# pzimbrod/fem-glass-tempering

Measured on AMD Instinct MI355X. Metric: DOF-updates/sec (coupled thermo-visco time step, 3D CG1 hex), higher is better.
Workload: dtype f64; 1 GPU; C4 3D plate CG1/CG1 400x400x50 hex (8200851 T-dofs), dt 0.1, coupled 6-term Prony; parallelism=single GPU, one partition (no communication), output=none (reference writes VTX/XDMF every step), krylov_form=PETSc KSPCG, geometric-multigrid V-cycle preconditioner, preconditioner=gmg, visco_fields=state (T, Tf, Tf_partial, phi, xi, s_tilde, sigma_tilde, sigma)

## Files before the change

fem-glass-tempering_amd/csrc/tv_cg.hip:

```cpp
#include <algorithm>
#include <cstdlib>

#include "tv_stencil.h"


#include <cstdio>
#include <vector>

namespace tv {
namespace {


using buf_t = __amdgpu_buffer_rsrc_t;
using b64v = unsigned int __attribute__((ext_vector_type(2)));
constexpr uint32_t kBadOff = 0x40000000u;
__device__ __forceinline__ buf_t mk_rsrc(const void* p, uint32_t bytes) {
  const uint64_t a = (uint64_t)p;
  const uint32_t lo = __builtin_amdgcn_readfirstlane((uint32_t)a);
  const uint32_t hi = __builtin_amdgcn_readfirstlane((uint32_t)(a >> 32));
  void* q = (void*)(((uint64_t)hi << 32) | lo);
  return __builtin_amdgcn_make_buffer_rsrc(q, (short)0, (int)__builtin_amdgcn_readfirstlane(bytes), 0x00020000);
}
__device__ __forceinline__ double bload(buf_t r, uint32_t off) {
  return __builtin_bit_cast(double, __builtin_amdgcn_raw_buffer_load_b64(r, (int)off, 0, 0));
}
__device__ __forceinline__ void bstore(buf_t r, uint32_t off, double v) {
  __builtin_amdgcn_raw_buffer_store_b64(__builtin_bit_cast(b64v, v), r, (int)off, 0, 0);
}

__device__ __forceinline__ double uniform(double v) {
  const int lo = __builtin_amdgcn_readfirstlane(__double2loint(v));
  const int hi = __builtin_amdgcn_readfirstlane(__double2hiint(v));
  return __hiloint2double(hi, lo);
}

__device__ __forceinline__ double wave_sum(double v) {
#pragma unroll
  for (int off = 32; off >= 1; off >>= 1) v += __shfl_xor(v, off, 64);
  return v;
}


template <int DIM, int MODE, bool FUSEP>
__global__ __launch_bounds__(kBlock) void k_cg_rows(CgGrid g, const double* __restrict__ T,
                                                    const double* __restrict__ in0,
                                                    const double* in1,
                                                    double* __restrict__ out, double* pout,
                                                    const PcgState* __restrict__ st,
                                                    double* __restrict__ partials, int nseg, int kfirst,
                                                    int nplanes, int wmode) {
  constexpr bool D1 = (DIM <= 2);
  constexpr bool D2 = (DIM == 1);
  __shared__ double red[kBlock / kWave];
  if (st != nullptr && st->done) return;
  const int lane = threadIdx.x & (kWave - 1);
  const int wave = threadIdx.x >> 6;
  int seg, j, kp;
  if (wmode == 0) {
    const int n1b = (g.n1 + 3) >> 2;
    const int b = blockIdx.x;
    seg = b % nseg;
    const int t = b / nseg;
    j = (t % n1b) * 4 + wave;
    kp = t / n1b;
  } else {
    const int gw = blockIdx.x * 4 + wave;
    seg = gw % nseg;
    const int row = gw / nseg;
    j = row % g.n1;
    kp = row / g.n1;
  }
  const int k = kfirst + kp;
  const bool row_ok = (j < g.n1) && (kp < nplanes);
  const int i = seg * kSeg - 1 + lane;
  const bool col_ok = row_ok && (i >= 0) && (i < g.n0);
  const int n0 = g.n0, n1 = g.n1, n2 = g.n2;
  const int64_t plane = (int64_t)n0 * n1;

  double bcoef = 0.0;
  bool first = false;
  const double* pold = in1;
  if (FUSEP) {
    const int it = st->it;
    first = (it == 0);
    bcoef = first ? 0.0 : st->beta / st->betaold;
    if (it & 1) {
      pold = in1;
    } else {
      pold = pout;
      pout = const_cast<double*>(in1);
    }
  }

  double X[3][3];
  double Mm[3][3];
#pragma unroll
  for (int b = 0; b < 3; ++b) {
#pragma unroll
    for (int c = 0; c < 3; ++c) {
      const int jj = j + b - 1, kk = k + c - 1;
      const bool ok = col_ok && (D1 ? b == 1 : (jj >= 0 && jj < n1)) && (D2 ? c == 1 : (kk >= 0 && kk < n2));
      const int64_t idx = (int64_t)i + (int64_t)n0 * jj + plane * kk;
      double v = 0.0, v2 = 0.0;
      if (ok) {
        v = in0[idx];
        if (MODE == MODE_RES) v2 = in1[idx];
        if (FUSEP) v = first ? v : v + bcoef * pold[idx];
      }
      X[b][c] = v;
      if (MODE == MODE_RES) Mm[b][c] = v - v2 - g.dt_f;
    }
  }
  const double* cy = g.coef[1] + (int64_t)(j < n1 ? j : 0) * C_NCOEF;
  const double* cz = g.coef[2] + (int64_t)(k < n2 ? k : 0) * C_NCOEF;
  const double My[3] = {cy[C_MLO], cy[C_MDI], cy[C_MUP]};
  const double Ky[3] = {cy[C_KLO], cy[C_KDI], cy[C_KUP]};
  const double Mz[3] = {cz[C_MLO], cz[C_MDI], cz[C_MUP]};
  const double Kz[3] = {cz[C_KLO], cz[C_KDI], cz[C_KUP]};
  const double da = g.dt_alpha;

  double S1 = 0.0, S2 = 0.0;
#pragma unroll
  for (int c = 0; c < 3; ++c) {
    double us = 0.0, vs = 0.0, um = 0.0;
#pragma unroll
    for (int b = 0; b < 3; ++b) {
      us += My[b] * X[b][c];
      vs += Ky[b] * X[b][c];
      if (MODE == MODE_RES) um += My[b] * Mm[b][c];
    }
    if (MODE != MODE_RES) um = us;
    S1 += Mz[c] * (um + da * vs) + da * Kz[c] * us;
    S2 += Mz[c] * us;
  }
  S2 *= da;

  const double S1m = shr1(S1), S1p = shl1(S1), S2m = shr1(S2), S2p = shl1(S2);
  const double* cx = g.coef[0] + (int64_t)(col_ok ? i : 0) * C_NCOEF;
  double y = 0.0;
  if (col_ok) {
    y = cx[C_MLO] * S1m + cx[C_MDI] * S1 + cx[C_MUP] * S1p + cx[C_KLO] * S2m + cx[C_KDI] * S2 +
        cx[C_KUP] * S2p;
  }

  if (!D2 && row_ok && ((k == 0 && g.bnd[2][0]) || (k == n2 - 1 && g.bnd[2][1]))) {
    double Tp_[3][3], Pp_[3][3];
#pragma unroll
    for (int v = 0; v < 3; ++v) {
      double pc = X[v][1], tc;
      if (MODE == MODE_RES) {
        tc = pc;
      } else {
        const int jj = j + v - 1;
        const bool ok = col_ok && (D1 ? v == 1 : (jj >= 0 && jj < n1));
        tc = ok ? T[(int64_t)i + (int64_t)n0 * jj + plane * k] : 0.0;
      }
      Tp_[0][v] = shr1(tc); Tp_[1][v] = tc; Tp_[2][v] = shl1(tc);
      Pp_[0][v] = shr1(pc); Pp_[1][v] = pc; Pp_[2][v] = shl1(pc);
    }
    if (col_ok) {
      y += facet_sum<MODE, false, false, D1>(g, cx[C_HLO], cx[C_HHI], cy[C_HLO], cy[C_HHI], Tp_, Pp_);
    }
  }
  if (!D1 && row_ok && ((j == 0 && g.bnd[1][0]) || (j == n1 - 1 && g.bnd[1][1]))) {
    double Tp_[3][3], Pp_[3][3];
#pragma unroll
    for (int v = 0; v < 3; ++v) {
      double pc = X[1][v], tc;
      if (MODE == MODE_RES) {
        tc = pc;
      } else {
        const int kk = k + v - 1;
        const bool ok = col_ok && (D2 ? v == 1 : (kk >= 0 && kk < n2));
        tc = ok ? T[(int64_t)i + (int64_t)n0 * j + plane * kk] : 0.0;
      }
      Tp_[0][v] = shr1(tc); Tp_[1][v] = tc; Tp_[2][v] = shl1(tc);
      Pp_[0][v] = shr1(pc); Pp_[1][v] = pc; Pp_[2][v] = shl1(pc);
    }
    if (col_ok) {
      y += facet_sum<MODE, false, false, D2>(g, cx[C_HLO], cx[C_HHI], cz[C_HLO], cz[C_HHI], Tp_, Pp_);
    }
  }
  if (col_ok && ((i == 0 && g.bnd[0][0]) || (i == n0 - 1 && g.bnd[0][1]))) {
    double Tp_[3][3];
    if (MODE == MODE_RES) {
#pragma unroll
      for (int u = 0; u < 3; ++u)
#pragma unroll
        for (int v = 0; v < 3; ++v) Tp_[u][v] = X[u][v];
    } else {
#pragma unroll
      for (int u = 0; u < 3; ++u) {
#pragma unroll
        for (int v = 0; v < 3; ++v) {
          const int jj = j + u - 1, kk = k + v - 1;
          const bool ok = (D1 ? u == 1 : (jj >= 0 && jj < n1)) && (D2 ? v == 1 : (kk >= 0 && kk < n2));
          Tp_[u][v] = ok ? T[(int64_t)i + (int64_t)n0 * jj + plane * kk] : 0.0;
        }
      }
    }
    y += facet_sum<MODE, false, D1, D2>(g, cy[C_HLO], cy[C_HHI], cz[C_HLO], cz[C_HHI], Tp_, X);
  }

  const bool owned = (k >= g.k_begin) && (k < g.k_end);
  const bool inwin = (k >= g.w_begin) && (k < g.w_end);
  const bool writer = col_ok && lane >= 1 && lane <= kSeg;
  const int64_t me = (int64_t)i + (int64_t)n0 * j + plane * k;
  if (writer) {
    if (FUSEP) pout[me] = X[1][1];
    if (inwin) out[me] = y;
  }
  if (MODE == MODE_JAC && partials != nullptr) {
    double d = (writer && owned) ? X[1][1] * y : 0.0;
    d = wave_sum(d);
    if (lane == 0) red[wave] = d;
    __syncthreads();
    if (threadIdx.x == 0) store_partial(&partials[blockIdx.x], (red[0] + red[1]) + (red[2] + red[3]));
  }
}


template <int DIM, bool FACETS>
__device__ __forceinline__ double diag_value(const CgGrid& g, const double* __restrict__ T, int64_t n) {
  constexpr bool D1 = (DIM <= 2);
  constexpr bool D2 = (DIM == 1);
  const int64_t plane = (int64_t)g.n0 * g.n1;
  int i, j, k;
  decode_node(n, g, i, j, k);
  const double* cx = g.coef[0] + (int64_t)i * C_NCOEF;
  const double* cy = g.coef[1] + (int64_t)j * C_NCOEF;
  const double* cz = g.coef[2] + (int64_t)k * C_NCOEF;
  double d = cx[C_MDI] * cy[C_MDI] * cz[C_MDI] +
             g.dt_alpha * (cx[C_KDI] * cy[C_MDI] * cz[C_MDI] + cx[C_MDI] * cy[C_KDI] * cz[C_MDI] +
                           cx[C_MDI] * cy[C_MDI] * cz[C_KDI]);
  if (!FACETS) return d;
  auto load_patch = [&](int64_t stride_a, int64_t stride_b, bool dega, bool degb, int ia, int na, int ib, int nb,
                        double (&P)[3][3]) {
#pragma unroll
    for (int u = 0; u < 3; ++u)
#pragma unroll
      for (int v = 0; v < 3; ++v) {
        const int aa = ia + u - 1, bb = ib + v - 1;
        const bool ok = (dega ? u == 1 : (aa >= 0 && aa < na)) && (degb ? v == 1 : (bb >= 0 && bb < nb));
        P[u][v] = ok ? T[n + (int64_t)(u - 1) * stride_a + (int64_t)(v - 1) * stride_b] : 0.0;
      }
  };
  double P[3][3];
  if ((i == 0 && g.bnd[0][0]) || (i == g.n0 - 1 && g.bnd[0][1])) {
    load_patch(g.n0, plane, D1, D2, j, g.n1, k, g.n2, P);
    d += facet_sum<MODE_JAC, true, D1, D2>(g, cy[C_HLO], cy[C_HHI], cz[C_HLO], cz[C_HHI], P, P);
  }
  if (!D1 && ((j == 0 && g.bnd[1][0]) || (j == g.n1 - 1 && g.bnd[1][1]))) {
    load_patch(1, plane, false, D2, i, g.n0, k, g.n2, P);
    d += facet_sum<MODE_JAC, true, false, D2>(g, cx[C_HLO], cx[C_HHI], cz[C_HLO], cz[C_HHI], P, P);
  }
  if (!D2 && ((k == 0 && g.bnd[2][0]) || (k == g.n2 - 1 && g.bnd[2][1]))) {
    load_patch(1, g.n0, false, D1, i, g.n0, j, g.n1, P);
    d += facet_sum<MODE_JAC, true, false, D1>(g, cx[C_HLO], cx[C_HHI], cy[C_HLO], cy[C_HHI], P, P);
  }
  return d;
}

template <int DIM, bool FACETS>
__global__ __launch_bounds__(kBlock) void k_cg_diag(CgGrid g, const double* __restrict__ T,
                                                    double* __restrict__ out, int invert) {
  const int64_t plane = (int64_t)g.n0 * g.n1;
  const int64_t nown = plane * (g.w_end - g.w_begin);
  const int64_t base = plane * g.w_begin;
  for (int64_t t = blockIdx.x * (int64_t)blockDim.x + threadIdx.x; t < nown;
       t += (int64_t)gridDim.x * blockDim.x) {
    const int64_t n = base + t;
    const double d = diag_value<DIM, FACETS>(g, T, n);
    out[n] = invert ? 1.0 / d : d;
  }
}

__global__ __launch_bounds__(kBlock) void k_cg_diag_bnd(CgGrid g, const double* __restrict__ T,
                                                        double* __restrict__ out, int invert) {
  for (int64_t t = blockIdx.x * (int64_t)blockDim.x + threadIdx.x; t < g.n_bnodes;
       t += (int64_t)gridDim.x * blockDim.x) {
    const int64_t n = g.bnodes[t];
    const double d = diag_value<3, true>(g, T, n);
    out[n] = invert ? 1.0 / d : d;
  }
}


constexpr int kRows = 8;
constexpr int kFaceChunk = 16;

template <int MODE, bool FUSEP>
__device__ double facet_direct(const CgGrid& g, int i, int j, int k, int ax, const double* __restrict__ T,
                               const double* __restrict__ in0, const double* pold, double bcoef, bool first) {
  const int t1 = (ax == 0) ? 1 : 0, t2 = (ax == 2) ? 1 : 2;
  const int c[3] = {i, j, k};
  const int n[3] = {g.n0, g.n1, g.n2};
  const int64_t st[3] = {1, g.n0, (int64_t)g.n0 * g.n1};
  const int64_t me = (int64_t)i + st[1] * j + st[2] * k;
  double Tp[3][3], Pp[3][3];
#pragma unroll
  for (int u = 0; u < 3; ++u)
#pragma unroll
    for (int v = 0; v < 3; ++v) {
      const int a = c[t1] + u - 1, b = c[t2] + v - 1;
      const bool ok = a >= 0 && a < n[t1] && b >= 0 && b < n[t2];
      const int64_t off = me + (int64_t)(u - 1) * st[t1] + (int64_t)(v - 1) * st[t2];
      if (MODE == MODE_RES) {
        Tp[u][v] = ok ? in0[off] : 0.0;
        Pp[u][v] = 0.0;
      } else {
        Tp[u][v] = ok ? T[off] : 0.0;
        double pv = ok ? in0[off] : 0.0;
        if (FUSEP && ok && !first) pv = pv + bcoef * pold[off];
        Pp[u][v] = pv;
      }
    }
  const double* c1 = g.coef[t1] + (int64_t)c[t1] * C_NCOEF;
  const double* c2 = g.coef[t2] + (int64_t)c[t2] * C_NCOEF;
  return facet_sum<MODE, false, false, false>(g, c1[C_HLO], c1[C_HHI], c2[C_HLO], c2[C_HHI], Tp, Pp);
}

struct FaceOff {
  int off[7];
};

FaceOff face_offsets(const CgGrid& g, int R, int qaxis) {
  FaceOff fo{};
  int acc = 0;
  const int rows = R - 1;
  for (int f = 0; f < 6; ++f) {
    fo.off[f] = acc;
    if (g.fface[f] && (f >> 1) != qaxis) acc += ((g.fn1[f] + kSeg - 1) / kSeg) * ((g.fn2[f] + rows - 1) / rows);
  }
  fo.off[6] = acc;
  return fo;
}

__device__ __forceinline__ void facet_corners(const CgGrid& g, bool ok, double h1, double h2, double Ta,
                                              double Tc, double Pa, double Pc, double& ya, double& yb,
                                              double& yc, double& yd) {
  const double Tb = shl1(Ta), Td = shl1(Tc), Pb = shl1(Pa), Pd = shl1(Pc);
  ya = yb = yc = yd = 0.0;
  if (ok) {
#pragma unroll
    for (int q1 = 0; q1 < 3; ++q1) {
#pragma unroll
      for (int q2 = 0; q2 < 3; ++q2) {
        const double sx = kGX[q1], tx = kGX[q2];
        const double fa = (1.0 - sx) * (1.0 - tx), fb = sx * (1.0 - tx), fc = (1.0 - sx) * tx, fd = sx * tx;
        const double Th = fa * Ta + fb * Tb + fc * Tc + fd * Td;
        const double Ph = fa * Pa + fb * Pb + fc * Pc + fd * Pd;
        const double G = (kGW[q1] * kGW[q2]) * dg_rad_conv(g, Th) * Ph;
        ya += G * fa;
        yb += G * fb;
        yc += G * fc;
        yd += G * fd;
      }
    }
    const double sc = g.dt * (h1 * h2);
    ya *= sc; yb *= sc; yc *= sc; yd *= sc;
  }
}

template <bool FUSEP, int R>
__device__ void face_block(const CgGrid& g, const double* __restrict__ T, const double* __restrict__ in0,
                           const double* pA, const double* pB, double beta_ratio,
                           double* __restrict__ partials, const RedTail& rt, int nrec, int fb,
                           const FaceOff& fo, double* sm, double* redf, int it_host) {
  double (*sT)[kWave] = reinterpret_cast<double (*)[kWave]>(sm);
  double (*sP)[kWave] = reinterpret_cast<double (*)[kWave]>(sm + (R + 1) * kWave);
  double (*sCD)[R][kWave] = reinterpret_cast<double (*)[R][kWave]>(sm + 2 * (R + 1) * kWave);
  int f = 0;
  while (f < 5 && fb >= fo.off[f + 1]) ++f;
  const int a = f >> 1, side = f & 1;
  const int t1 = (a == 0) ? 1 : 0, t2 = (a == 2) ? 1 : 2;
  const int n[3] = {g.n0, g.n1, g.n2};
  const int sst[3] = {1, g.n0, g.n0 * g.n1};
  const int n1 = n[t1], n2 = n[t2];
  const int nseg1 = (n1 + kSeg - 1) / kSeg;
  const int tile = fb - fo.off[f];
  const int seg = tile % nseg1, tb = tile / nseg1;
  const int lane = threadIdx.x & (kWave - 1);
  const int wave = __builtin_amdgcn_readfirstlane(threadIdx.x >> 6);
  const int c1 = seg * kSeg - 1 + lane;
  const int r0 = tb * (R - 1);
  const bool ok1 = c1 >= 0 && c1 < n1;
  double bcoef = 0.0;
  bool first = true;
  const double* pold = pA;
  if (FUSEP) {
    first = (it_host == 0);
    bcoef = first ? 0.0 : beta_ratio;
    pold = (it_host & 1) ? pA : pB;
  }
  auto node_of = [&](int cc1, int cc2) {
    int c[3];
    c[t1] = cc1;
    c[t2] = cc2;
    c[a] = side ? n[a] - 1 : 0;
    return c[0] + sst[1] * c[1] + sst[2] * c[2];
  };
  struct Stg {
    double tt, zz, oo;
    bool ok;
  };
  auto stage_ld = [&](int cc2) -> Stg {
    const bool ok = ok1 && cc2 >= 0 && cc2 < n2;
    const int o = ok ? node_of(c1, cc2) : 0;
    return Stg{T[o], in0[o], FUSEP ? pold[o] : 0.0, ok};
  };
  auto stage_st = [&](int row, const Stg& v) {
    sT[row][lane] = v.ok ? v.tt : 0.0;
    sP[row][lane] = v.ok ? ((FUSEP && !first) ? v.zz + bcoef * v.oo : v.zz) : 0.0;
  };
  const int fr = r0 - 1 + wave;
  const bool facet_ok = c1 >= 0 && c1 < n1 - 1 && fr >= 0 && fr < n2 - 1;
  const double h1 = g.coef[t1][(int64_t)(facet_ok ? c1 : 0) * C_NCOEF + C_HHI];
  const double h2 = g.coef[t2][(int64_t)(facet_ok ? fr : 0) * C_NCOEF + C_HHI];
  const Stg sa = stage_ld(r0 - 1 + wave);
  Stg sb{0.0, 0.0, 0.0, false};
  if (wave == R - 1) sb = stage_ld(r0 + R - 1);
  stage_st(wave, sa);
  if (wave == R - 1) stage_st(R, sb);
  __syncthreads();
  const double Pa = sP[wave][lane];
  double ya, yb, yc, yd;
  facet_corners(g, facet_ok, h1, h2, sT[wave][lane], sT[wave + 1][lane], Pa, sP[wave + 1][lane], ya, yb, yc, yd);
  sCD[0][wave][lane] = yc;
  sCD[1][wave][lane] = yd;
  const double ybl = shr1(yb);
  __syncthreads();
  double dot = 0.0;
  const int c2 = r0 - 1 + wave;
  const bool wr = wave >= 1 && ok1 && lane >= 1 && lane <= kSeg && c2 < n2;
  if (wr) {
    const double acc = (ya + ybl) + (sCD[0][wave - 1][lane] + sCD[1][wave - 1][lane - 1]);
    int c[3];
    c[t1] = c1;
    c[t2] = c2;
    c[a] = side ? n[a] - 1 : 0;
    const bool owned = c[2] >= g.k_begin && c[2] < g.k_end;
    g.fface[f][c1 + n1 * c2] = (c[2] >= g.w_begin && c[2] < g.w_end) ? acc : 0.0;
    dot = owned ? Pa * acc : 0.0;
  }
  if (partials != nullptr) {
    dot = wave_sum(dot);
    if (lane == 0) redf[wave] = dot;
    __syncthreads();
    if (threadIdx.x == 0) {
      double s2 = 0.0;
#pragma unroll
      for (int w = 0; w < R; ++w) s2 += redf[w];
      store_partial(&partials[blockIdx.x], s2);
    }
    fused_reduce_tail<1>(rt, nrec);
  }
}

__global__ __launch_bounds__(kBlock) void k_cg_addfaces(CgGrid g, double* __restrict__ out, int raxis,
                                                        const PcgState* __restrict__ st) {
  if (st != nullptr && st->done) return;
  const int n[3] = {g.n0, g.n1, g.n2};
  const int kb = g.w_begin, nk = g.w_end - g.w_begin;
  const int sx = n[0] > 1 ? 2 : 1;
  const int64_t nA = (int64_t)sx * n[1] * nk;
  const int nin = n[0] - 2 > 0 ? n[0] - 2 : 0;
  const int nfree = (raxis == 1) ? nk : n[1];
  const int64_t nB = 2 * (int64_t)nin * nfree;
  const double* fb = nullptr;
#pragma unroll
  for (int f = 0; f < 6; ++f)
    if (fb == nullptr && g.fface[f] != nullptr) fb = g.fface[f] - g.ffoff[f];
  const buf_t rsF = mk_rsrc(fb, fb ? (uint32_t)(g.ffsize * 8) : 0u);
  const uint32_t obytes = (uint32_t)n[0] * (uint32_t)n[1] * (uint32_t)n[2] * 8u;
  const buf_t rsO = mk_rsrc(out, obytes);
  const int fr_lo = (raxis == 1) ? 2 : 4;
  for (int64_t e = blockIdx.x * (int64_t)kBlock + threadIdx.x; e < nA + nB; e += (int64_t)gridDim.x * kBlock) {
    int c[3];
    if (e < nA) {
      const int64_t pl = (int64_t)n[1] * nk;
      const int side = (int)(e / pl);
      const int64_t r = e - side * pl;
      c[0] = side ? n[0] - 1 : 0;
      c[1] = (int)(r % n[1]);
      c[2] = kb + (int)(r / n[1]);
    } else {
      const int64_t u = e - nA, pl = (int64_t)nin * nfree;
      const int side = (int)(u / pl);
      const int64_t r = u - side * pl;
      c[0] = 1 + (int)(r % nin);
      const int o = (int)(r / nin);
      if (raxis == 1) {
        c[1] = side ? n[1] - 1 : 0;
        c[2] = kb + o;
      } else {
        c[1] = o;
        c[2] = side ? n[2] - 1 : 0;
        if (c[2] < kb || c[2] >= g.w_end) continue;
      }
    }
    const bool x0 = g.fface[0] && c[0] == 0, x1 = g.fface[1] && c[0] == n[0] - 1;
    const bool r0 = g.fface[fr_lo] && c[raxis] == 0, r1 = g.fface[fr_lo + 1] && c[raxis] == n[raxis] - 1;
    const int rt2 = (raxis == 1) ? c[2] : c[1];
    const int64_t ex = (x0 ? g.ffoff[0] : g.ffoff[1]) + c[1] + (int64_t)n[1] * c[2];
    const int64_t er = (r0 ? g.ffoff[fr_lo] : g.ffoff[fr_lo + 1]) + c[0] + (int64_t)n[0] * rt2;
    const uint32_t oq = (uint32_t)(c[0] + (int64_t)n[0] * (c[1] + (int64_t)n[1] * c[2])) * 8u;
    const double fx = bload(rsF, (x0 || x1) ? (uint32_t)ex * 8u : kBadOff);
    const double fr = bload(rsF, (r0 || r1) ? (uint32_t)er * 8u : kBadOff);
    const double old = bload(rsO, oq);
    const double add = fx + fr;
    if (add != 0.0) bstore(rsO, oq, old + add);
  }
}

__device__ __forceinline__ void march_tile(int bid, int nmarch, int nseg, int nrbk, int nch, int& seg, int& rb,
                                           int& chunk) {
  const int x = bid & 7, p = bid >> 3;
  const int q = nmarch >> 3, r = nmarch & 7;
  const int start = x * q + min(x, r);
  const int per_chunk = nseg * nrbk;
  const int nF = (nch > 1 ? 2 : 1) * per_chunk;
  const int fq = nF >> 3, fr = nF & 7;
  const int fsize = fq + (x < fr ? 1 : 0), fstart = x * fq + min(x, fr);
  int t, c;
  if (p < fsize) {
    t = fstart + p;
    c = t / per_chunk;
    chunk = c ? nch - 1 : 0;
  } else {
    t = (start - fstart) + (p - fsize);
    c = t / per_chunk;
    chunk = 1 + c;
  }
  t -= c * per_chunk;
  seg = t % nseg;
  rb = t / nseg;
}

template <int MODE, bool FUSEP, int R, int WPE, int PF, bool POST = false>
__global__ __launch_bounds__(R * kWave) __attribute__((amdgpu_waves_per_eu(WPE))) void k_cg_march(CgGrid g, const double* __restrict__ T,
                                                        const double* __restrict__ in0, const double* in1,
                                                        double* __restrict__ out, double* pout,
                                                        const PcgState* __restrict__ st,
                                                        double* __restrict__ partials, int nseg, int raxis,
                                                        int qchunk, RedTail rt, int nrec, int nmarch,
                                                        FaceOff fo, int it_host, PostArgs pa) {
  static_assert(!POST || (MODE == MODE_JAC && !FUSEP), "POST: plain Jacobian march only");
  stamp_start(rt);
  constexpr int NA = (MODE == MODE_RES) ? 2 : 1;
  __shared__ double lds[NA][2][R + 2][kWave];
  __shared__ double red[R];
  constexpr int kFaceLds = (MODE == MODE_JAC) ? (8 * R + 8) * kWave : 1;
  __shared__ double fsm[kFaceLds];
  const int bid = (int)blockIdx.x;
  const int fidx = (MODE == MODE_JAC && bid >= nmarch) ? bid - nmarch : -1;
  const bool lagged = FUSEP && rt.lag != nullptr;
  if (lagged && bid == 0 && threadIdx.x == 0) {
    const PcgState s = lagged_state(st, rt.lag, rt.lag_kind);
    if (s.done) *rt.st = s;
  }
  if (fidx >= 0) {
    double ratio = 0.0;
    if (lagged) {
      int ldone;
      double lbeta;
      lag_update_lean(st, rt.lag, ldone, lbeta);
      if (ldone) return;
      ratio = lbeta / st->betaold;
    } else if (st != nullptr) {
      if (st->done) return;
      if (FUSEP) ratio = st->beta / st->betaold;
    }
    face_block<FUSEP, R>(g, T, in0, in1, pout, ratio, POST ? nullptr : partials, POST ? RedTail{} : rt, nrec, fidx, fo,
                         fsm, red, it_host);
    return;
  }
  const int lane = threadIdx.x & (kWave - 1);
  const int wave = __builtin_amdgcn_readfirstlane(threadIdx.x >> 6);
  const int n0 = g.n0;
  const int nR = (raxis == 1) ? g.n1 : g.n2;
  const int nQ = (raxis == 1) ? g.n2 : g.n1;
  const int64_t sR = (raxis == 1) ? (int64_t)n0 : (int64_t)n0 * g.n1;
  const int64_t sQ = (raxis == 1) ? (int64_t)n0 * g.n1 : (int64_t)n0;
  const int nch = (nQ + qchunk - 1) / qchunk;
  const int nrbk = (nR + R - 1) / R;
  int seg, rb, chunk;
  march_tile(bid, nmarch, nseg, nrbk, nch, seg, rb, chunk);
  const int r0 = rb * R;
  const int r = r0 + wave;
  const bool row_ok = r < nR;
  const int q0 = chunk * qchunk;
  const int q1 = min(q0 + qchunk, nQ);
  const int i = seg * kSeg - 1 + lane;
  const bool col_ok = (i >= 0) && (i < n0);
  const bool writer = col_ok && lane >= 1 && lane <= kSeg;

  double bcoef = 0.0;
  bool first = false;
  const double* pold = in1;
  if (FUSEP) {
    first = (it_host == 0);
    if (!(it_host & 1)) { pold = pout; pout = const_cast<double*>(in1); }
  }
  int st_done = 0;
  double st_beta = 0.0, st_betaold = 1.0;
  if (lagged) {
    lag_update_lean(st, rt.lag, st_done, st_beta);
    st_done = __builtin_amdgcn_readfirstlane(st_done);
    st_beta = uniform(st_beta);
    st_betaold = st->betaold;
  } else if (st != nullptr) {
    st_done = st->done;
    if (FUSEP) {
      st_beta = st->beta;
      st_betaold = st->betaold;
    }
  }
  const int kb = g.k_begin, ke = g.k_end, wb = g.w_begin, we = g.w_end;
  const bool row_owned = (raxis == 2) ? (r >= kb && r < ke) : true;
  const bool row_inwin = (raxis == 2) ? (r >= wb && r < we) : true;
  const double* coefR = (raxis == 1) ? g.coef[1] : g.coef[2];
  const double* coefQ = (raxis == 1) ? g.coef[2] : g.coef[1];
  const int bq_lo = (raxis == 1) ? g.bnd[2][0] : g.bnd[1][0];
  const int bq_hi = (raxis == 1) ? g.bnd[2][1] : g.bnd[1][1];

  const bool fq0 = (MODE == MODE_JAC) && q0 == 0 && bq_lo;
  const bool fq1 = (MODE == MODE_JAC) && q1 == nQ && bq_hi;
  double (*sFq)[2][R + 2][kWave] = reinterpret_cast<double (*)[2][R + 2][kWave]>(fsm);
  double (*sCD)[2][R][kWave] = reinterpret_cast<double (*)[2][R][kWave]>(fsm + 4 * (R + 2) * kWave);
  double yq0 = 0.0, yq1 = 0.0;
  const double da = g.dt_alpha;

  const double* second = (MODE == MODE_RES) ? in1 : pold;
  constexpr bool TWO = (MODE == MODE_RES) || FUSEP;
  const uint32_t nbytes = (uint32_t)g.n0 * (uint32_t)g.n1 * (uint32_t)g.n2 * 8u;
  const buf_t rs0 = mk_rsrc(in0, nbytes);
  const buf_t rs1 = mk_rsrc(TWO ? second : in0, (FUSEP && first) ? 0u : nbytes);
  const buf_t rso = mk_rsrc(out, nbytes);
  const buf_t rsp = mk_rsrc(FUSEP ? pout : out, FUSEP ? nbytes : 0u);
  const buf_t rsT = mk_rsrc(T, (fq0 || fq1) ? nbytes : 0u);
  const buf_t rsZ = mk_rsrc(in0, (fq0 || fq1) ? nbytes : 0u);
  const buf_t rsO = mk_rsrc(TWO ? second : in0, ((fq0 || fq1) && FUSEP && !first) ? nbytes : 0u);
  const bool halo = (wave == 0) || (wave == R - 1);
  const int hrow = (wave == 0) ? r0 - 1 : (wave == R - 1 ? r0 + R : r);
  const int hslot = (wave == 0) ? 0 : R + 1;
  auto lane_off = [&](int rr) -> uint32_t {
    return (col_ok && rr >= 0 && rr < nR) ? (uint32_t)(i + sR * rr) * 8u : kBadOff;
  };
  const uint32_t vo_own = lane_off(r), vo_halo = halo ? lane_off(hrow) : kBadOff;
  const uint32_t vo_wr = writer ? vo_own : kBadOff;
  auto plane_off = [&](int L) -> uint32_t { return (L >= 0 && L < nQ) ? (uint32_t)(sQ * L) * 8u : kBadOff; };
  auto fetch = [&](uint32_t vo, int L, double& a0, double& a1) {
    const uint32_t o = vo + plane_off(L);
    a0 = bload(rs0, o);
    a1 = TWO ? bload(rs1, o) : 0.0;
  };
  const buf_t rsr = mk_rsrc(pa.r, POST ? nbytes : 0u);
  const buf_t rsd = mk_rsrc(pa.dinv, POST ? nbytes : 0u);
  const int bR_lo = (raxis == 1) ? g.bnd[1][0] : g.bnd[2][0], bR_hi = (raxis == 1) ? g.bnd[1][1] : g.bnd[2][1];
  const bool bnd_lr = (i == 0) || (i == n0 - 1) || (r == 0 && bR_lo) || (r == nR - 1 && bR_hi);
  auto bnd_q = [&](int q) { return (q == 0 && bq_lo) || (q == nQ - 1 && bq_hi); };
  auto fetch_post = [&](int L, double& a_r, double& a_d) {
    if (!POST) return;
    const uint32_t o = vo_wr + plane_off(L - 1);
    a_r = bload(rsr, o);
    a_d = bload(rsd, (bnd_lr || bnd_q(L - 1)) ? o : kBadOff);
  };

  auto combine = [&](uint32_t vo, int L, double a0, double a1, double& v, double& vm) {
    v = a0;
    vm = 0.0;
    if (MODE == MODE_RES) vm = (vo != kBadOff && L >= 0 && L < nQ) ? a0 - a1 - g.dt_f : 0.0;
    if (FUSEP) v = a0 + bcoef * a1;
  };
  double ra0[PF + 1], ra1[PF + 1], rh0[PF + 1], rh1[PF + 1];
  double rr[PF + 1], rd[PF + 1];
#pragma unroll
  for (int s = 0; s < PF; ++s) {
    fetch(vo_own, q0 - 1 + s, ra0[s], ra1[s]);
    fetch(vo_halo, q0 - 1 + s, rh0[s], rh1[s]);
    fetch_post(q0 - 1 + s, rr[s], rd[s]);
  }
  __shared__ double2 cql[kFaceChunk + 2][5];
  __shared__ double2 cxl[4][kWave];
  __shared__ double crl[R + 1][C_NCOEF];
  const int nqs = q1 - q0 + 2;
  const bool st_q = (int)threadIdx.x < nqs * 6;
  const bool st_x = (int)threadIdx.x < 8 * kWave;
  const bool st_r = (int)threadIdx.x < (R + 1) * C_NCOEF;
  double cqv, cxv, crv;
  {
    const int e = threadIdx.x;
    const int qq = q0 - 1 + e / 6;
    const bool okq = st_q && qq >= 0 && qq < nQ;
    cqv = coefQ[okq ? (int64_t)qq * C_NCOEF + e % 6 : 0];
    const int ii = seg * kSeg - 1 + (e & (kWave - 1));
    const bool okx = st_x && ii >= 0 && ii < n0;
    const int k = e >> 6;
    const int cc = k == 0 ? C_MLO : k == 1 ? C_KLO : k == 2 ? C_MDI : k == 3 ? C_KDI : k == 4 ? C_MUP : k == 5 ? C_KUP : C_HHI;
    cxv = g.coef[0][okx ? (int64_t)ii * C_NCOEF + cc : 0];
    const int rrow = r0 - 1 + e / C_NCOEF;
    const bool okr = st_r && rrow >= 0 && rrow < nR;
    crv = coefR[okr ? (int64_t)rrow * C_NCOEF + e % C_NCOEF : 0];
    cqv = okq ? cqv : 0.0;
    cxv = (okx && k < 7) ? cxv : 0.0;
    crv = okr ? crv : 0.0;
  }
  double fT[2][2], fZ[2][2], fO[2][2];
  if (fq0 || fq1) {
#pragma unroll
    for (int f = 0; f < 2; ++f) {
      const uint32_t po = plane_off(f == 0 ? (fq0 ? 0 : -1) : (fq1 ? nQ - 1 : -1));
      fT[f][0] = bload(rsT, vo_own + po); fT[f][1] = bload(rsT, vo_halo + po);
      fZ[f][0] = bload(rsZ, vo_own + po); fZ[f][1] = bload(rsZ, vo_halo + po);
      fO[f][0] = FUSEP ? bload(rsO, vo_own + po) : 0.0;
      fO[f][1] = FUSEP ? bload(rsO, vo_halo + po) : 0.0;
    }
  }
  if (st_done) return;
  if (FUSEP) bcoef = first ? 0.0 : st_beta / st_betaold;
  if (st_q) {
    const int qs = threadIdx.x / 6, c = threadIdx.x % 6;
    double* row = reinterpret_cast<double*>(cql[qs]);
    if (c < 3) {
      row[c] = cqv;
      row[6 + c] = da * cqv;
    } else {
      row[c] = da * cqv;
    }
    if (c == 0) row[9] = 0.0;
  }
  if (st_x) reinterpret_cast<double*>(cxl[(threadIdx.x >> 6) >> 1])[2 * (threadIdx.x & (kWave - 1)) + ((threadIdx.x >> 6) & 1)] = cxv;
  if (st_r) crl[threadIdx.x / C_NCOEF][threadIdx.x % C_NCOEF] = crv;
  if (fq0 || fq1) {
#pragma unroll
    for (int f = 0; f < 2; ++f) {
      sFq[f][0][wave + 1][lane] = fT[f][0];
      sFq[f][1][wave + 1][lane] = FUSEP ? fZ[f][0] + bcoef * fO[f][0] : fZ[f][0];
      if (halo) {
        sFq[f][0][hslot][lane] = fT[f][1];
        sFq[f][1][hslot][lane] = FUSEP ? fZ[f][1] + bcoef * fO[f][1] : fZ[f][1];
      }
    }
  }
  __syncthreads();
  const double* crw = crl[wave + 1];
  const double My0 = uniform(crw[C_MLO]), My1 = uniform(crw[C_MDI]), My2 = uniform(crw[C_MUP]);
  const double Ky0 = uniform(crw[C_KLO]), Ky1 = uniform(crw[C_KDI]), Ky2 = uniform(crw[C_KUP]);
  const double hq_own = uniform(crw[C_HHI]);
  const double hq_low = uniform(crl[0][C_HHI]);
  if (fq0 || fq1) {
    const bool cok = i >= 0 && i < n0 - 1;
    const double h1 = cxl[3][lane].x;
#pragma unroll
    for (int f = 0; f < 2; ++f) {
      if (!(f == 0 ? fq0 : fq1)) continue;
      double ya, yb, yc, yd;
      facet_corners(g, cok && r < nR - 1, h1, hq_own, sFq[f][0][wave + 1][lane], sFq[f][0][wave + 2][lane],
                    sFq[f][1][wave + 1][lane], sFq[f][1][wave + 2][lane], ya, yb, yc, yd);
      double yq = ya + shr1(yb);
      sCD[f][0][wave][lane] = yc;
      sCD[f][1][wave][lane] = yd;
      if (wave == 0) {
        facet_corners(g, cok && r0 >= 1 && r0 - 1 < nR - 1, h1, hq_low, sFq[f][0][0][lane], sFq[f][0][1][lane],
                      sFq[f][1][0][lane], sFq[f][1][1][lane], ya, yb, yc, yd);
        yq += yc + shr1(yd);
      }
      if (f == 0) yq0 = yq; else yq1 = yq;
    }
    __syncthreads();
    if (wave >= 1) {
      const int lm = lane >= 1 ? lane - 1 : 0;
      yq0 += sCD[0][0][wave - 1][lane] + sCD[0][1][wave - 1][lm];
      yq1 += sCD[1][0][wave - 1][lane] + sCD[1][1][wave - 1][lm];
    }
  }

  double us_m = 0.0, us_c = 0.0, t_m = 0.0, t_c = 0.0;
  double xc = 0.0;
  double dot = 0.0, zz = 0.0, zr = 0.0;
  auto step = [&](int L, double c0, double c1, double h0, double h1, double pr, double pd) {
    const int buf = L & 1;
    double v, vm;
    combine(vo_own, L, c0, c1, v, vm);
    if (FUSEP) bstore(rsp, vo_wr + ((L >= q0 && L < q1) ? plane_off(L) : kBadOff), v);
    lds[0][buf][wave + 1][lane] = v;
    if (MODE == MODE_RES) lds[NA - 1][buf][wave + 1][lane] = vm;
    if (halo) {
      double hv, hvm;
      combine(vo_halo, L, h0, h1, hv, hvm);
      lds[0][buf][hslot][lane] = hv;
      if (MODE == MODE_RES) lds[NA - 1][buf][hslot][lane] = hvm;
    }
    __syncthreads();
    const double x0 = lds[0][buf][wave][lane], x1 = v, x2 = lds[0][buf][wave + 2][lane];
    const double us_p = My0 * x0 + My1 * x1 + My2 * x2;
    const double vs_p = Ky0 * x0 + Ky1 * x1 + Ky2 * x2;
    double um_p = us_p;
    if (MODE == MODE_RES) um_p = My0 * lds[NA - 1][buf][wave][lane] + My1 * vm + My2 * lds[NA - 1][buf][wave + 2][lane];
    const double t_p = um_p + da * vs_p;
    if (L >= q0 + 1 && L <= q1) {
      const int q = L - 1;
      const double2* cq = cql[q - q0 + 1];
      const double2 c01 = cq[0], c23 = cq[1], c45 = cq[2], c67 = cq[3], c89 = cq[4];
      const double S1 = c01.x * t_m + c01.y * t_c + c23.x * t_p + (c23.y * us_m + c45.x * us_c + c45.y * us_p);
      const double S2 = c67.x * us_m + c67.y * us_c + c89.x * us_p;
      const double2 xlo = cxl[0][lane], xdi = cxl[1][lane], xup = cxl[2][lane];
      const double Lt = xup.x * S1 + xup.y * S2;
      const double Rt = xlo.x * S1 + xlo.y * S2;
      const double y = (xdi.x * S1 + xdi.y * S2) + (shr1(Lt) + shl1(Rt));
      const bool q_owned = (raxis == 2) ? true : (q >= kb && q < ke);
      const bool q_inwin = (raxis == 2) ? true : (q >= wb && q < we);
      const bool wr = writer && row_ok && row_owned && q_owned;
      const bool inwin = row_inwin && q_inwin;
      double yb = y;
      if (fq0 && q == 0) yb += yq0;
      if (fq1 && q == nQ - 1) yb += yq1;
      if (POST) {
        const double xm = xdi.x, xk = xdi.y;
        const double dI = xm * My1 * c01.y + ((xk * My1 * c67.y + xm * Ky1 * c67.y) + xm * My1 * c45.x);
        const double dq = (bnd_lr || bnd_q(q)) ? pd : 1.0 / dI;
        const double zq = xc + pa.omega * dq * (pr - yb);
        bstore(rso, inwin ? vo_wr + plane_off(q) : kBadOff, zq);
        zz += wr ? zq * zq : 0.0;
        zr += wr ? zq * pr : 0.0;
      } else {
        bstore(rso, inwin ? vo_wr + plane_off(q) : kBadOff, yb);
      }
      if (MODE == MODE_JAC && !POST) dot += wr ? xc * yb : 0.0;
    }
    xc = x1;
    us_m = us_c; us_c = us_p;
    t_m = t_c; t_c = t_p;
  };
  for (int L = q0 - 1; L <= q1; L += PF + 1) {
#pragma unroll
    for (int s = 0; s <= PF; ++s) {
      const int sf = (s + PF) % (PF + 1);
      fetch(vo_own, L + s + PF, ra0[sf], ra1[sf]);
      fetch(vo_halo, L + s + PF, rh0[sf], rh1[sf]);
      fetch_post(L + s + PF, rr[sf], rd[sf]);
      step(L + s, ra0[s], ra1[s], rh0[s], rh1[s], POST ? rr[s] : 0.0, POST ? rd[s] : 0.0);
    }
  }
  if (POST) {
    zz = wave_sum(zz);
    zr = wave_sum(zr);
    if (lane == 0) {
      red[wave] = zz;
      fsm[wave] = zr;
    }
    __syncthreads();
    if (threadIdx.x == 0) {
      double a = 0.0, c = 0.0;
#pragma unroll
      for (int w = 0; w < R; ++w) {
        a += red[w];
        c += fsm[w];
      }
      store_partial(&partials[2 * (int64_t)bid], a);
      store_partial(&partials[2 * (int64_t)bid + 1], c);
    }
    return;
  }
  if (MODE == MODE_JAC && partials != nullptr) {
    dot = wave_sum(dot);
    if (lane == 0) red[wave] = dot;
    __syncthreads();
    if (threadIdx.x == 0) {
      double s = 0.0;
#pragma unroll
      for (int w = 0; w < R; ++w) s += red[w];
      store_partial(&partials[blockIdx.x], s);
    }
    fused_reduce_tail<1>(rt, nrec);
  }
}


__device__ __forceinline__ uint32_t ff_off_x(const CgGrid& g, int i, int j, int k) {
  const int f = (i == 0) ? 0 : (i == g.n0 - 1 ? 1 : -1);
  if (f < 0 || g.ffoff[f] < 0) return kBadOff;
  return (uint32_t)(g.ffoff[f] + j + (int64_t)g.n1 * k) * 8u;
}
__device__ __forceinline__ uint32_t ff_off_r(const CgGrid& g, int ra, int i, int j, int k) {
  const int c = (ra == 1) ? j : k, n = (ra == 1) ? g.n1 : g.n2;
  const int side = (c == 0) ? 0 : (c == n - 1 ? 1 : -1);
  if (side < 0 || i < 0 || i >= g.n0) return kBadOff;
  const int f = 2 * ra + side;
  if (g.ffoff[f] < 0) return kBadOff;
  return (uint32_t)(g.ffoff[f] + i + (int64_t)g.n0 * ((ra == 1) ? k : j)) * 8u;
}

struct CgsScal {
  double a, b;
  bool first;
};

template <bool INIT>
__device__ __forceinline__ void cgs_node(const CgsScal& k, double R, double S, double W, double D, double ff,
                                         double& s, double& r, double& u) {
  if (INIT) {
    s = 0.0;
    r = R;
  } else {
    const double wf = W + ff;
    s = k.first ? wf : wf + k.b * S;
    r = R - k.a * s;
  }
  u = D * r;
}

template <bool INIT, int R>
__device__ void face_block_cgs(const CgGrid& g, const CgsBuffers& v, const CgsScal& ks, int raxis,
                               double* __restrict__ partials, int fb, const FaceOff& fo, double* sm,
                               double (*red)[R]) {
  double (*sT)[kWave] = reinterpret_cast<double (*)[kWave]>(sm);
  double (*sP)[kWave] = reinterpret_cast<double (*)[kWave]>(sm + (R + 1) * kWave);
  double (*sCD)[R][kWave] = reinterpret_cast<double (*)[R][kWave]>(sm + 2 * (R + 1) * kWave);
  int f = 0;
  while (f < 5 && fb >= fo.off[f + 1]) ++f;
  const int a = f >> 1, side = f & 1;
  const int t1 = (a == 0) ? 1 : 0, t2 = (a == 2) ? 1 : 2;
  const int n[3] = {g.n0, g.n1, g.n2};
  const int n1 = n[t1], n2 = n[t2];
  const int nseg1 = (n1 + kSeg - 1) / kSeg;
  const int tile = fb - fo.off[f];
  const int seg = tile % nseg1, tb = tile / nseg1;
  const int lane = threadIdx.x & (kWave - 1);
  const int wave = __builtin_amdgcn_readfirstlane(threadIdx.x >> 6);
  const int c1 = seg * kSeg - 1 + lane;
  const int r0 = tb * (R - 1);
  const bool ok1 = c1 >= 0 && c1 < n1;
  const buf_t rsFin = mk_rsrc(v.fin, (uint32_t)(g.ffsize * 8));
  struct Stg {
    double tt, R_, D, S, W, fx, fr;
    bool ok;
  };
  auto stage_ld = [&](int cc2) -> Stg {
    Stg q{};
    q.ok = ok1 && cc2 >= 0 && cc2 < n2;
    int c[3];
    c[t1] = q.ok ? c1 : 0;
    c[t2] = q.ok ? cc2 : 0;
    c[a] = side ? n[a] - 1 : 0;
    const int64_t o = c[0] + (int64_t)g.n0 * c[1] + (int64_t)g.n0 * g.n1 * c[2];
    q.tt = v.T[o];
    q.R_ = v.rin[o];
    q.D = v.dinv[o];
    if (!INIT) {
      q.S = ks.first ? 0.0 : v.sin[o];
      q.W = v.win[o];
      q.fx = bload(rsFin, ff_off_x(g, c[0], c[1], c[2]));
      q.fr = bload(rsFin, ff_off_r(g, raxis, c[0], c[1], c[2]));
    }
    return q;
  };
  auto stage_st = [&](int row, const Stg& q) {
    double s, r, u;
    cgs_node<INIT>(ks, q.R_, q.S, q.W, q.D, INIT ? 0.0 : q.fx + q.fr, s, r, u);
    sT[row][lane] = q.ok ? q.tt : 0.0;
    sP[row][lane] = q.ok ? u : 0.0;
  };
  const int fr = r0 - 1 + wave;
  const bool facet_ok = c1 >= 0 && c1 < n1 - 1 && fr >= 0 && fr < n2 - 1;
  const double h1 = g.coef[t1][(int64_t)(facet_ok ? c1 : 0) * C_NCOEF + C_HHI];
  const double h2 = g.coef[t2][(int64_t)(facet_ok ? fr : 0) * C_NCOEF + C_HHI];
  const Stg sa = stage_ld(r0 - 1 + wave);
  Stg sb{};
  if (wave == R - 1) sb = stage_ld(r0 + R - 1);
  stage_st(wave, sa);
  if (wave == R - 1) stage_st(R, sb);
  __syncthreads();
  const double Pa = sP[wave][lane];
  double ya, yb, yc, yd;
  facet_corners(g, facet_ok, h1, h2, sT[wave][lane], sT[wave + 1][lane], Pa, sP[wave + 1][lane], ya, yb, yc, yd);
  sCD[0][wave][lane] = yc;
  sCD[1][wave][lane] = yd;
  const double ybl = shr1(yb);
  __syncthreads();
  double dot = 0.0;
  const int c2 = r0 - 1 + wave;
  const bool wr = wave >= 1 && ok1 && lane >= 1 && lane <= kSeg && c2 < n2;
  if (wr) {
    const double acc = (ya + ybl) + (sCD[0][wave - 1][lane] + sCD[1][wave - 1][lane - 1]);
    int c[3];
    c[t1] = c1;
    c[t2] = c2;
    c[a] = side ? n[a] - 1 : 0;
    const bool owned = c[2] >= g.k_begin && c[2] < g.k_end;
    v.fout[g.ffoff[f] + c1 + (int64_t)n1 * c2] = owned ? acc : 0.0;
    dot = owned ? Pa * acc : 0.0;
  }
  dot = wave_sum(dot);
  if (lane == 0) red[1][wave] = dot;
  __syncthreads();
  if (threadIdx.x == 0) {
    double s2 = 0.0;
#pragma unroll
    for (int w = 0; w < R; ++w) s2 += red[1][w];
    store_partial(&partials[(int64_t)blockIdx.x * 3 + 0], 0.0);
    store_partial(&partials[(int64_t)blockIdx.x * 3 + 1], s2);
    store_partial(&partials[(int64_t)blockIdx.x * 3 + 2], 0.0);
  }
}

template <bool INIT, int R, int PF>
__global__ __launch_bounds__(R * kWave) void k_cgs_march(CgGrid g, CgsBuffers v, PcgState* __restrict__ st,
                                                         double* __restrict__ partials, int nseg, int raxis,
                                                         int qchunk, RedTail rt, int nrec, int nmarch, FaceOff fo,
                                                         int it_host, const double* __restrict__ lag_sums) {
  stamp_start(rt);
  __shared__ double lds[2][R + 2][kWave];
  __shared__ double red[3][R];
  constexpr int kFaceLds = (8 * R + 8) * kWave;
  __shared__ double fsm[kFaceLds];
  __shared__ PcgState sst;
  CgsScal ks{0.0, 0.0, it_host == 1};
  int st_done = 0;
  if (lag_sums != nullptr) {
    if (threadIdx.x == 0) {
      sst = *st;
      apply_logic(&sst, lag_sums, it_host == 1 ? 4 : 5);
    }
    __syncthreads();
    if (sst.done) {
      if (blockIdx.x == 0 && threadIdx.x == 0 && !st->done) *st = sst;
      return;
    }
    ks.a = sst.a;
    ks.b = sst.beta;
  } else if (!INIT) {
    st_done = st->done;
    ks.a = st->a;
    ks.b = st->beta;
  }
  const int nface = (int)gridDim.x - nmarch;
  if ((int)blockIdx.x >= nmarch && nface > 0) {
    if (st_done) return;
    face_block_cgs<INIT, R>(g, v, ks, raxis, partials, (int)blockIdx.x - nmarch, fo, fsm, red);
    cgs_tail(rt, nrec, st, lag_sums != nullptr ? &sst : nullptr);
    return;
  }
  const int lane = threadIdx.x & (kWave - 1);
  const int wave = __builtin_amdgcn_readfirstlane(threadIdx.x >> 6);
  const int n0 = g.n0;
  const int nR = (raxis == 1) ? g.n1 : g.n2;
  const int nQ = (raxis == 1) ? g.n2 : g.n1;
  const int64_t sR = (raxis == 1) ? (int64_t)n0 : (int64_t)n0 * g.n1;
  const int64_t sQ = (raxis == 1) ? (int64_t)n0 * g.n1 : (int64_t)n0;
  const int nrbk = (nR + R - 1) / R;
  int seg, rb, chunk;
  march_tile((int)blockIdx.x, nmarch, nseg, nrbk, (nQ + qchunk - 1) / qchunk, seg, rb, chunk);
  const int r0 = rb * R;
  const int r = r0 + wave;
  const bool row_ok = r < nR;
  const int q0 = chunk * qchunk;
  const int q1 = min(q0 + qchunk, nQ);
  const int i = seg * kSeg - 1 + lane;
  const bool col_ok = (i >= 0) && (i < n0);
  const bool writer = col_ok && lane >= 1 && lane <= kSeg;
  const int kb = g.k_begin, ke = g.k_end;
  const bool row_owned = (raxis == 2) ? (r >= kb && r < ke) : true;

  const double* coefR = (raxis == 1) ? g.coef[1] : g.coef[2];
  const double* coefQ = (raxis == 1) ? g.coef[2] : g.coef[1];
  const int bq_lo = (raxis == 1) ? g.bnd[2][0] : g.bnd[1][0];
  const int bq_hi = (raxis == 1) ? g.bnd[2][1] : g.bnd[1][1];
  const bool fq0 = q0 == 0 && bq_lo;
  const bool fq1 = q1 == nQ && bq_hi;
  double (*sFq)[2][R + 2][kWave] = reinterpret_cast<double (*)[2][R + 2][kWave]>(fsm);
  double (*sCD)[2][R][kWave] = reinterpret_cast<double (*)[2][R][kWave]>(fsm + 4 * (R + 2) * kWave);
  double yq0 = 0.0, yq1 = 0.0;
  const double da = g.dt_alpha;

  const uint32_t nbytes = (uint32_t)g.n0 * (uint32_t)g.n1 * (uint32_t)g.n2 * 8u;
  const buf_t rsR = mk_rsrc(v.rin, nbytes);
  const buf_t rsD = mk_rsrc(v.dinv, nbytes);
  const buf_t rsS = mk_rsrc(v.sin, (INIT || ks.first) ? 0u : nbytes);
  const buf_t rsW = mk_rsrc(v.win, INIT ? 0u : nbytes);
  const buf_t rsF = mk_rsrc(v.fin, INIT ? 0u : (uint32_t)g.ffsize * 8u);
  const buf_t rsP = mk_rsrc(v.p, (INIT || ks.first) ? 0u : nbytes);
  const buf_t rsX = mk_rsrc(v.x, (INIT || ks.first) ? 0u : nbytes);
  const buf_t wsR = mk_rsrc(v.rout, INIT ? 0u : nbytes);
  const buf_t wsS = mk_rsrc(v.sout, INIT ? 0u : nbytes);
  const buf_t wsP = mk_rsrc(v.p, INIT ? 0u : nbytes);
  const buf_t wsX = mk_rsrc(v.x, nbytes);
  const buf_t wsW = mk_rsrc(v.wout, nbytes);
  const buf_t rsT = mk_rsrc(v.T, (fq0 || fq1) ? nbytes : 0u);
  const bool halo = (wave == 0) || (wave == R - 1);
  const int hrow = (wave == 0) ? r0 - 1 : (wave == R - 1 ? r0 + R : r);
  const int hslot = (wave == 0) ? 0 : R + 1;
  auto lane_off = [&](int rr) -> uint32_t {
    return (col_ok && rr >= 0 && rr < nR) ? (uint32_t)(i + sR * rr) * 8u : kBadOff;
  };
  const uint32_t vo_own = lane_off(r), vo_halo = halo ? lane_off(hrow) : kBadOff;
  const uint32_t vo_wr = writer ? vo_own : kBadOff;
  auto plane_off = [&](int L) -> uint32_t { return (L >= 0 && L < nQ) ? (uint32_t)(sQ * L) * 8u : kBadOff; };
  auto xf_base = [&](int rr) -> int64_t {
    if (!col_ok || rr < 0 || rr >= nR) return -1;
    const int f = (i == 0) ? 0 : (i == n0 - 1 ? 1 : -1);
    return (f < 0) ? -1 : g.ffoff[f];
  };
  auto rf_base = [&](int rr) -> int64_t {
    if (!col_ok) return -1;
    const int f = (rr == 0) ? 2 * raxis : (rr == nR - 1 ? 2 * raxis + 1 : -1);
    return (f < 0) ? -1 : g.ffoff[f];
  };
  const int64_t xb_own = xf_base(r), rb_own = rf_base(r);
  const int64_t xb_hal = halo ? xf_base(hrow) : -1, rb_hal = halo ? rf_base(hrow) : -1;
  auto ff_offs = [&](int64_t xb, int64_t rbse, int rr, int L, uint32_t& ox, uint32_t& orr) {
    const bool okL = L >= 0 && L < nQ;
    const int64_t ix = (raxis == 2) ? ((int64_t)L + (int64_t)g.n1 * rr) : ((int64_t)rr + (int64_t)g.n1 * L);
    ox = (xb >= 0 && okL) ? (uint32_t)(xb + ix) * 8u : kBadOff;
    orr = (rbse >= 0 && okL) ? (uint32_t)(rbse + i + (int64_t)n0 * L) * 8u : kBadOff;
  };

  struct Raw { double Rv, Sv, Wv, Dv, FX, FR, Pv, Xv; };
  auto fetch = [&](uint32_t vo, int64_t xb, int64_t rbse, int rr, int L, Raw& a, bool own) {
    const uint32_t o = vo + plane_off(L);
    a.Rv = bload(rsR, o);
    a.Dv = bload(rsD, o);
    a.Pv = a.Xv = 0.0;
    if (!INIT && own) {
      a.Pv = bload(rsP, o);
      a.Xv = bload(rsX, o);
    }
    if (!INIT) {
      a.Sv = bload(rsS, o);
      a.Wv = bload(rsW, o);
      uint32_t ox, orr;
      ff_offs(xb, rbse, rr, L, ox, orr);
      a.FX = bload(rsF, ox);
      a.FR = bload(rsF, orr);
    } else {
      a.Sv = a.Wv = a.FX = a.FR = 0.0;
    }
  };
  Raw ra[PF + 1], rh[PF + 1] = {};
#pragma unroll
  for (int sI = 0; sI < PF; ++sI) {
    fetch(vo_own, xb_own, rb_own, r, q0 - 1 + sI, ra[sI], true);
    if (halo) fetch(vo_halo, xb_hal, rb_hal, hrow, q0 - 1 + sI, rh[sI], false);
  }
  __shared__ double2 cql[kFaceChunk + 2][5];
  __shared__ double2 cxl[4][kWave];
// ... 575 lines not shown
```

Baseline: 837.9 million DOF-updates/s.

## Peel march loop into specialized steady-state body with scalar-offset buffer ops

The plane-marching CG stencil kernel gets a prologue, a steady-state loop and an epilogue. The steady-state body drops the per-plane bounds checks, boundary-face terms and window predicates, and addresses memory through wave-uniform scalar offsets (soffset) on the buffer loads and stores, which cuts VALU address arithmetic and branching per plane. The waves-per-EU hint also gets a default of 7 or 6 when WPE is 1, which limits register use. Risks are register pressure from three unrolled bodies plus a static_assert that ties the code to PF==2.

```diff
diff --git a/fem-glass-tempering_amd/csrc/tv_cg.hip b/fem-glass-tempering_amd/csrc/tv_cg.hip
--- a/fem-glass-tempering_amd/csrc/tv_cg.hip
+++ b/fem-glass-tempering_amd/csrc/tv_cg.hip
@@ -1,5 +1,6 @@
 #include <algorithm>
 #include <cstdlib>
+#include <type_traits>
 
 #include "tv_stencil.h"
 
@@ -26,6 +27,13 @@
 }
 __device__ __forceinline__ void bstore(buf_t r, uint32_t off, double v) {
   __builtin_amdgcn_raw_buffer_store_b64(__builtin_bit_cast(b64v, v), r, (int)off, 0, 0);
+}
+
+__device__ __forceinline__ double bload_s(buf_t r, uint32_t off, uint32_t soff) {
+  return __builtin_bit_cast(double, __builtin_amdgcn_raw_buffer_load_b64(r, (int)off, (int)soff, 0));
+}
+__device__ __forceinline__ void bstore_s(buf_t r, uint32_t off, uint32_t soff, double v) {
+  __builtin_amdgcn_raw_buffer_store_b64(__builtin_bit_cast(b64v, v), r, (int)off, (int)soff, 0);
 }
 
 __device__ __forceinline__ double uniform(double v) {
@@ -538,7 +546,7 @@
 }
 
 template <int MODE, bool FUSEP, int R, int WPE, int PF, bool POST = false>
-__global__ __launch_bounds__(R * kWave) __attribute__((amdgpu_waves_per_eu(WPE))) void k_cg_march(CgGrid g, const double* __restrict__ T,
+__global__ __launch_bounds__(R * kWave) __attribute__((amdgpu_waves_per_eu(WPE > 1 ? WPE : (MODE == MODE_RES ? 7 : 6)))) void k_cg_march(CgGrid g, const double* __restrict__ T,
                                                         const double* __restrict__ in0, const double* in1,
                                                         double* __restrict__ out, double* pout,
                                                         const PcgState* __restrict__ st,
@@ -667,10 +675,10 @@
     a_d = bload(rsd, (bnd_lr || bnd_q(L - 1)) ? o : kBadOff);
   };
 
-  auto combine = [&](uint32_t vo, int L, double a0, double a1, double& v, double& vm) {
+  auto combine = [&](bool in_dom, double a0, double a1, double& v, double& vm) {
     v = a0;
     vm = 0.0;
-    if (MODE == MODE_RES) vm = (vo != kBadOff && L >= 0 && L < nQ) ? a0 - a1 - g.dt_f : 0.0;
+    if (MODE == MODE_RES) vm = in_dom ? a0 - a1 - g.dt_f : 0.0;
     if (FUSEP) v = a0 + bcoef * a1;
   };
   double ra0[PF + 1], ra1[PF + 1], rh0[PF + 1], rh1[PF + 1];
@@ -679,7 +687,7 @@
   for (int s = 0; s < PF; ++s) {
     fetch(vo_own, q0 - 1 + s, ra0[s], ra1[s]);
     fetch(vo_halo, q0 - 1 + s, rh0[s], rh1[s]);
-    fetch_post(q0 - 1 + s, rr[s], rd[s]);
+    rr[s] = rd[s] = 0.0;
   }
   __shared__ double2 cql[kFaceChunk + 2][5];
   __shared__ double2 cxl[4][kWave];
@@ -779,18 +787,40 @@
   double us_m = 0.0, us_c = 0.0, t_m = 0.0, t_c = 0.0;
   double xc = 0.0;
   double dot = 0.0, zz = 0.0, zr = 0.0;
-  auto step = [&](int L, double c0, double c1, double h0, double h1, double pr, double pd) {
+  constexpr int S_GEN = 1, S_NOPST = 2, S_NOOUT = 4;
+  const uint32_t sQ8 = (uint32_t)sQ * 8u;
+  const bool own_in = vo_own != kBadOff, halo_in = vo_halo != kBadOff;
+  const bool wr_row = writer && row_ok && row_owned;
+  const uint32_t vo_st = row_inwin ? vo_wr : kBadOff;
+  const uint32_t vo_dq = bnd_lr ? vo_wr : kBadOff;
+  const int hs_any = halo ? hslot : wave + 1;
+  auto step = [&](auto flags, int L, uint32_t pc, double c0, double c1, double h0, double h1, double pr, double pd) {
+    constexpr int F = decltype(flags)::value;
+    constexpr bool GEN = (F & S_GEN) != 0;
+    const bool l_in = !GEN || (L >= 0 && L < nQ);
     const int buf = L & 1;
     double v, vm;
-    combine(vo_own, L, c0, c1, v, vm);
-    if (FUSEP) bstore(rsp, vo_wr + ((L >= q0 && L < q1) ? plane_off(L) : kBadOff), v);
-    lds[0][buf][wave + 1][lane] = v;
-    if (MODE == MODE_RES) lds[NA - 1][buf][wave + 1][lane] = vm;
-    if (halo) {
+    combine(own_in && l_in, c0, c1, v, vm);
+    if (FUSEP) {
+      if (!GEN) bstore_s(rsp, vo_wr, pc, v);
+      else if (!(F & S_NOPST)) bstore(rsp, vo_wr + ((L >= q0 && L < q1) ? plane_off(L) : kBadOff), v);
+    }
+    if (GEN) {
+      lds[0][buf][wave + 1][lane] = v;
+      if (MODE == MODE_RES) lds[NA - 1][buf][wave + 1][lane] = vm;
+      if (halo) {
+        double hv, hvm;
+        combine(halo_in && l_in, h0, h1, hv, hvm);
+        lds[0][buf][hslot][lane] = hv;
+        if (MODE == MODE_RES) lds[NA - 1][buf][hslot][lane] = hvm;
+      }
+    } else {
       double hv, hvm;
-      combine(vo_halo, L, h0, h1, hv, hvm);
-      lds[0][buf][hslot][lane] = hv;
-      if (MODE == MODE_RES) lds[NA - 1][buf][hslot][lane] = hvm;
+      combine(halo_in && l_in, h0, h1, hv, hvm);
+      lds[0][buf][hs_any][lane] = hv;
+      if (MODE == MODE_RES) lds[NA - 1][buf][hs_any][lane] = hvm;
+      lds[0][buf][wave + 1][lane] = v;
+      if (MODE == MODE_RES) lds[NA - 1][buf][wave + 1][lane] = vm;
     }
     __syncthreads();
     const double x0 = lds[0][buf][wave][lane], x1 = v, x2 = lds[0][buf][wave + 2][lane];
@@ -799,8 +829,9 @@
     double um_p = us_p;
     if (MODE == MODE_RES) um_p = My0 * lds[NA - 1][buf][wave][lane] + My1 * vm + My2 * lds[NA - 1][buf][wave + 2][lane];
     const double t_p = um_p + da * vs_p;
-    if (L >= q0 + 1 && L <= q1) {
+    if (!GEN || (!(F & S_NOOUT) && L >= q0 + 1 && L <= q1)) {
       const int q = L - 1;
+      constexpr bool FACE = GEN;
       const double2* cq = cql[q - q0 + 1];
       const double2 c01 = cq[0], c23 = cq[1], c45 = cq[2], c67 = cq[3], c89 = cq[4];
       const double S1 = c01.x * t_m + c01.y * t_c + c23.x * t_p + (c23.y * us_m + c45.x * us_c + c45.y * us_p);
@@ -809,23 +840,29 @@
       const double Lt = xup.x * S1 + xup.y * S2;
       const double Rt = xlo.x * S1 + xlo.y * S2;
       const double y = (xdi.x * S1 + xdi.y * S2) + (shr1(Lt) + shl1(Rt));
-      const bool q_owned = (raxis == 2) ? true : (q >= kb && q < ke);
-      const bool q_inwin = (raxis == 2) ? true : (q >= wb && q < we);
-      const bool wr = writer && row_ok && row_owned && q_owned;
+      const bool q_owned = (!GEN || raxis == 2) ? true : (q >= kb && q < ke);
+      const bool q_inwin = (!GEN || raxis == 2) ? true : (q >= wb && q < we);
+      const bool wr = wr_row && q_owned;
       const bool inwin = row_inwin && q_inwin;
+      auto put = [&](double val) {
+        if (GEN) bstore(rso, inwin ? vo_wr + plane_off(q) : kBadOff, val);
+        else bstore_s(rso, vo_st, pc - sQ8, val);
+      };
       double yb = y;
-      if (fq0 && q == 0) yb += yq0;
-      if (fq1 && q == nQ - 1) yb += yq1;
+      if (FACE && fq0 && q == 0) yb += yq0;
+      if (FACE && fq1 && q == nQ - 1) yb += yq1;
       if (POST) {
         const double xm = xdi.x, xk = xdi.y;
         const double dI = xm * My1 * c01.y + ((xk * My1 * c67.y + xm * Ky1 * c67.y) + xm * My1 * c45.x);
-        const double dq = (bnd_lr || bnd_q(q)) ? pd : 1.0 / dI;
+        const bool bnd = bnd_lr || (FACE && bnd_q(q));
+        const double inv = 1.0 / (bnd ? 1.0 : dI);
+        const double dq = bnd ? pd : inv;
         const double zq = xc + pa.omega * dq * (pr - yb);
-        bstore(rso, inwin ? vo_wr + plane_off(q) : kBadOff, zq);
+        put(zq);
         zz += wr ? zq * zq : 0.0;
         zr += wr ? zq * pr : 0.0;
       } else {
-        bstore(rso, inwin ? vo_wr + plane_off(q) : kBadOff, yb);
+        put(yb);
       }
       if (MODE == MODE_JAC && !POST) dot += wr ? xc * yb : 0.0;
     }
@@ -833,15 +870,51 @@
     us_m = us_c; us_c = us_p;
     t_m = t_c; t_c = t_p;
   };
-  for (int L = q0 - 1; L <= q1; L += PF + 1) {
-#pragma unroll
-    for (int s = 0; s <= PF; ++s) {
-      const int sf = (s + PF) % (PF + 1);
-      fetch(vo_own, L + s + PF, ra0[sf], ra1[sf]);
-      fetch(vo_halo, L + s + PF, rh0[sf], rh1[sf]);
-      fetch_post(L + s + PF, rr[sf], rd[sf]);
-      step(L + s, ra0[s], ra1[s], rh0[s], rh1[s], POST ? rr[s] : 0.0, POST ? rd[s] : 0.0);
-    }
+  static_assert(PF == 2, "the peeled march unrolls three register sets");
+  auto one = [&](auto flags, auto set, int L, uint32_t pc) {
+    constexpr int s = decltype(set)::value, sf = (s + PF) % (PF + 1);
+    if (decltype(flags)::value & S_GEN) {
+      fetch(vo_own, L + PF, ra0[sf], ra1[sf]);
+      fetch(vo_halo, L + PF, rh0[sf], rh1[sf]);
+      fetch_post(L + PF, rr[sf], rd[sf]);
+    } else {
+      const uint32_t po = pc + 2u * sQ8;
+      ra0[sf] = bload_s(rs0, vo_own, po);
+      ra1[sf] = TWO ? bload_s(rs1, vo_own, po) : 0.0;
+      rh0[sf] = bload_s(rs0, vo_halo, po);
+      rh1[sf] = TWO ? bload_s(rs1, vo_halo, po) : 0.0;
+      if (POST) {
+        rr[sf] = bload_s(rsr, vo_wr, pc + sQ8);
+        rd[sf] = bload_s(rsd, vo_dq, pc + sQ8);
+      }
+    }
+    step(flags, L, pc, ra0[s], ra1[s], rh0[s], rh1[s], POST ? rr[s] : 0.0, POST ? rd[s] : 0.0);
+  };
+  using std::integral_constant;
+  constexpr integral_constant<int, 0> i0{};
+  constexpr integral_constant<int, 1> i1{};
+  constexpr integral_constant<int, 2> i2{};
+  constexpr integral_constant<int, S_GEN> gen{};
+  int L = q0 - 1;
+  one(integral_constant<int, S_GEN | S_NOPST | S_NOOUT>{}, i0, L, 0u);
+  one(integral_constant<int, S_GEN | S_NOOUT>{}, i1, L + 1, 0u);
+  one(gen, i2, L + 2, 0u);
+  L += 3;
+  const bool q_all = (raxis == 2) || (q0 >= kb && q1 <= ke && q0 >= wb && q1 <= we);
+  const int trips = q_all ? (q1 - q0 - 4) / 3 : 0;
+  uint32_t pc = (uint32_t)__builtin_amdgcn_readfirstlane((int)(sQ8 * (uint32_t)L));
+  for (int t = trips; t > 0; --t) {
+    asm volatile("; march-isa: steady-state");
+    one(i0, i0, L, pc);
+    one(i0, i1, L + 1, pc + sQ8);
+    one(i0, i2, L + 2, pc + 2u * sQ8);
+    L += 3;
+    pc += 3u * sQ8;
+  }
+  for (; L <= q1; L += PF + 1) {
+    one(gen, i0, L, 0u);
+    one(gen, i1, L + 1, 0u);
+    one(gen, i2, L + 2, 0u);
   }
   if (POST) {
     zz = wave_sum(zz);
```

Result: no change. 843.3 million DOF-updates/s, median of 6 (+0.6%).
